# zhenpeiyang/RelativePose

Hardware: AMD Instinct MI355X
Metric: scan-pairs/sec end-to-end (completion+feat+spectral-match), 160x640 RGB-D (higher is better)
Workload: dtype f32 (fp32 products emulated on the bf16 matrix pipe: every operand cut into 3 bf16 pieces = its full 24 significand bits, the 6 partial products >= 2^-16 |ab| issued as v_mfma_f32_32x32x16_bf16, the 3 smallest dropped: a product error <= 2^-23 |ab| worst case, rms 2^-27.4 -- an fp32 multiply's own r

## Files before the change

include/relpose.h:

```cpp
#ifndef RELPOSE_H
#define RELPOSE_H

#include <stddef.h>
#include <stdint.h>

#ifdef __cplusplus
extern "C" {
#endif

#define RELPOSE_EINVAL (-1)
#define RELPOSE_ENOMEM (-2)
#define RELPOSE_EROUNDS (-3)

enum {
    RELPOSE_OK = 0,
    RELPOSE_FEW_KEYPOINTS = 1,
    RELPOSE_DIST_FILTER = 2,
    RELPOSE_ANGLE_FILTER = 3,
    RELPOSE_ZERO_WEIGHT = 4,
    RELPOSE_EDGE_OVERFLOW = 5,
    RELPOSE_NOT_CONVERGED = 6
};

enum { RELPOSE_SUNCG = 0, RELPOSE_MATTERPORT = 1, RELPOSE_SCANNET = 2 };
// ... 3 lines not shown

typedef struct RelposeParams {
    double distThre;
    double distSepThre;
    double angleThre;
    double sigmaAngle1, sigmaAngle2, sigmaDist, sigmaFeat;
    double mu;
    int32_t topK;
    int32_t method;
} RelposeParams;

void relpose_default_params(RelposeParams* p_host);

enum { RELPOSE_TUNE_AFFINITY_KERNEL = 0, RELPOSE_TUNE_FIT_MAX_PRODUCTS = 1, RELPOSE_TUNE_FIT_CLUSTER = 2,
       RELPOSE_TUNE_FIT_GLOBAL_VECTORS = 3, RELPOSE_TUNE_FIT_FIXED_CHECKS = 4, RELPOSE_TUNE_HEADS_KERNEL = 5, RELPOSE_TUNE_DECONV_STRIP = 6,
       RELPOSE_TUNE_ZERO_TILES = 7, RELPOSE_TUNE_CONV1_ZERO = 8, RELPOSE_TUNE_CONV4_ROWS = 9, RELPOSE_TUNE_COUNT = 10 };
int relpose_set_tuning(int32_t key, int32_t value);
const char* relpose_version(void);
typedef struct RelposeKeypoints {
    int32_t B, ns_max, nt_max;
    const int32_t* ns;
    const int32_t* nt;
    const double* pc_s;
    const double* normal_s;
    const float* feat_s;
    const double* weight_s;
    const double* pc_t;
    const double* normal_t;
    const float* feat_t;
    const double* weight_t;
} RelposeKeypoints;
// ... 716 lines not shown
} RelposeForwardArgs;
int relpose_scnet_forward_ex(RelposeSCNet* net, const RelposeForwardArgs* args);

int relpose_scnet_last_tail(RelposeSCNet* net);

int relpose_scnet_plan_macs(RelposeSCNet* net, int32_t n_images, int32_t flags, int32_t self_cached, double* macs_host);

int relpose_scnet_layer_kernel(RelposeSCNet* net, const char* layer, int32_t n_images);

int relpose_scnet_zero_tiles(RelposeSCNet* net, void* workspace, void* stream, int64_t* counts_host);

int relpose_scnet_conv1_zero(RelposeSCNet* net, void* workspace, void* stream, int64_t* counts_host, uint32_t* occ_host);

int relpose_scnet_conv4_rows(RelposeSCNet* net, void* workspace, void* stream, int64_t* counts_host);

int64_t relpose_scnet_read_tap(RelposeSCNet* net, const char* layer, float* out, void* workspace, void* stream);

int relpose_scnet_profile(RelposeSCNet* net, const float* x, float* out, int32_t n_images, int32_t H, int32_t W,
                          void* workspace, size_t workspace_bytes, int32_t iters,
                          double* ms_gemm_host, double* ms_other_host, int64_t* n_gemm_launches_host, void* stream);

#ifdef __cplusplus
}
#endif
#endif
```

relativepose_amd/_lib.py:

```python
import ctypes as C
import os

HERE = os.path.dirname(os.path.abspath(__file__))
LIB_PATH = os.environ.get("RELPOSE_LIB_PATH") or os.path.join(HERE, "librelpose_hip.so")

c_void_p, c_int, c_int64, c_size_t, c_double, c_char_p = C.c_void_p, C.c_int32, C.c_int64, C.c_size_t, C.c_double, C.c_char_p


class Params(C.Structure):
    _fields_ = [("distThre", c_double), ("distSepThre", c_double), ("angleThre", c_double),
                ("sigmaAngle1", c_double), ("sigmaAngle2", c_double), ("sigmaDist", c_double),
                ("sigmaFeat", c_double), ("mu", c_double), ("topK", c_int), ("method", c_int)]


class Keypoints(C.Structure):
    _fields_ = [("B", c_int), ("ns_max", c_int), ("nt_max", c_int),
                ("ns", c_void_p), ("nt", c_void_p),
                ("pc_s", c_void_p), ("normal_s", c_void_p), ("feat_s", c_void_p), ("weight_s", c_void_p),
                ("pc_t", c_void_p), ("normal_t", c_void_p), ("feat_t", c_void_p), ("weight_t", c_void_p)]


class MatchDebug(C.Structure):
    _fields_ = [("wij", c_void_p), ("corres_j", c_void_p), ("corres_w", c_void_p),
                ("counts", c_void_p), ("trace", c_void_p), ("eig_iters", c_void_p)]
# ... 301 lines not shown
    "relpose_scnet_create_ex": (c_void_p, [C.POINTER(SCNetConfig)]),
    "relpose_scnet_destroy": (None, [c_void_p]),
    "relpose_scnet_set_param": (c_int, [c_void_p, c_char_p, c_void_p, c_size_t]),
    "relpose_scnet_finalize": (c_int, [c_void_p]),
    "relpose_scnet_set_precision": (c_int, [c_void_p, c_int]),
    "relpose_scnet_num_params": (c_int64, [c_void_p]),
    "relpose_scnet_workspace_bytes": (c_size_t, [c_void_p, c_int, c_int, c_int]),
    "relpose_scnet_forward": (c_int, [c_void_p, c_void_p, c_void_p, c_int, c_int, c_int, c_void_p, c_size_t, c_void_p]),
    "relpose_scnet_forward_ex": (c_int, [c_void_p, C.POINTER(ForwardArgs)]),
    "relpose_scnet_plan_macs": (c_int, [c_void_p, c_int, c_int, c_int, C.POINTER(c_double)]),
    "relpose_scnet_layer_kernel": (c_int, [c_void_p, c_char_p, c_int]),
    "relpose_scnet_zero_tiles": (c_int, [c_void_p, c_void_p, c_void_p, C.POINTER(c_int64)]),
    "relpose_scnet_last_tail": (c_int, [c_void_p]),
    "relpose_scnet_conv1_zero": (c_int, [c_void_p, c_void_p, c_void_p, C.POINTER(c_int64), c_void_p]),
    "relpose_scnet_conv4_rows": (c_int, [c_void_p, c_void_p, c_void_p, C.POINTER(c_int64)]),
    "relpose_scnet_read_tap": (c_int64, [c_void_p, c_char_p, c_void_p, c_void_p, c_void_p]),
    "relpose_scnet_profile": (c_int, [c_void_p, c_void_p, c_void_p, c_int, c_int, c_int, c_void_p, c_size_t, c_int,
                                      C.POINTER(c_double), C.POINTER(c_double), C.POINTER(c_int64), c_void_p]),
}

_lib = None


def lib():
    global _lib
    if _lib is None:
        if not os.path.exists(LIB_PATH):
            _build_locked()
        if not os.path.exists(LIB_PATH):
            raise RuntimeError(f"{LIB_PATH} not built: run `python -m relativepose_amd.build` "
# ... 13 lines not shown
def _build_locked():
    import fcntl
    from . import build as _b
    if not os.path.exists(os.environ.get("HIPCC", "/opt/rocm/bin/hipcc")):
        return
    with open(LIB_PATH + ".lock", "w") as lk:
        fcntl.flock(lk, fcntl.LOCK_EX)
        try:
            if not os.path.exists(LIB_PATH):
                _b.build(verbose=False)
        finally:
            fcntl.flock(lk, fcntl.LOCK_UN)


TUNE_KEYS = {"affinity_kernel": 0, "fit_max_products": 1, "fit_cluster": 2, "fit_global_vectors": 3, "fit_fixed_checks": 4,
             "heads_kernel": 5, "deconv_strip": 6, "zero_tiles": 7, "conv1_zero": 8, "conv4_rows": 9}
AFFINITY_KERNELS = {"auto": 0, "rows": 1, "tile": 2, "lds": 3, "pool": 4}


class tuning:

    def __init__(self, **kw):
        self.kw = {k: (AFFINITY_KERNELS[v] if k == "affinity_kernel" and isinstance(v, str) else int(v)) for k, v in kw.items()}
        self.old = {}

    def __enter__(self):
        for k, v in self.kw.items():
            self.old[k] = lib().relpose_set_tuning(TUNE_KEYS[k], v)
        return self

    def __exit__(self, *exc):
# ... 25 lines not shown
```

relativepose_amd/csrc/scnet.hip:

```cpp
#include "common.h"
#include "matcher_internal.h"
#include "conv1_zero_geom.h"
#include "sample_pixels.h"
#include <map>
#include <string>
#include <vector>
#include <algorithm>
#include <math.h>
#include <stdio.h>
#include <string.h>
#include <type_traits>
#include <stdlib.h>
#include <stddef.h>

namespace {

typedef float floatx16 __attribute__((ext_vector_type(16)));
typedef __bf16 bf16x8 __attribute__((ext_vector_type(8)));
typedef __bf16 bf16x4 __attribute__((ext_vector_type(4)));
typedef _Float16 f16x8 __attribute__((ext_vector_type(8)));
typedef _Float16 f16x4 __attribute__((ext_vector_type(4)));
template <int SPLIT> struct SplitT { typedef bf16x8 v8; typedef bf16x4 v4; };
template <> struct SplitT<2> { typedef f16x8 v8; typedef f16x4 v4; };
template <> struct SplitT<3> { typedef f16x8 v8; typedef f16x4 v4; };
// ... 501 lines not shown
#pragma unroll
            for (int i = 0; i < MI; ++i)
#pragma unroll
                for (int j = 0; j < NI; ++j) {
                    acc[i][j] = __builtin_amdgcn_mfma_f32_32x32x2f32(a[i].x, b[j].x, acc[i][j], 0, 0, 0);
                    acc[i][j] = __builtin_amdgcn_mfma_f32_32x32x2f32(a[i].y, b[j].y, acc[i][j], 0, 0, 0);
                    acc[i][j] = __builtin_amdgcn_mfma_f32_32x32x2f32(a[i].z, b[j].z, acc[i][j], 0, 0, 0);
                    acc[i][j] = __builtin_amdgcn_mfma_f32_32x32x2f32(a[i].w, b[j].w, acc[i][j], 0, 0, 0);
                }
        }
    } else rp_split_mma<SPLIT, MI, NI>(acc, At, a_rows, Bt, b_rows);
}

#define RP_DT_SPLIT_OCC 2
#define RP_DT_OCC(MI_, NI_, NW_, SP_, PAIR_) ((SP_) >= 4 ? 2 : ((MI_) * (NI_) == 1 ? ((NW_) == 4 ? (((SP_) && (PAIR_)) ? RP_DT_SPLIT_OCC : 3) : 2) : 2))
template <int MI, int NI, int NW, int TC, bool PAIR = false, int SPLIT = 0>
__global__ __launch_bounds__(NW * 64, RP_DT_OCC(MI, NI, NW, SPLIT, PAIR)) void deconv_tile_kernel(const ConvDesc* __restrict__ descs) {
    constexpr int NT = NW * 64, TR = 32 / TC;
    constexpr int LD = RowLd<SPLIT>::v;
    constexpr bool S3 = SPLIT >= 4;
    constexpr int WB = S3 ? 6 : 4;
    constexpr int PR = PAIR ? 8 : (TC == 16 ? TR * MI * NW : TR), PW = PAIR ? 8 : (TC == 16 ? 16 : TC * NW), HW2 = PW + 2;
    constexpr int SUBPIX = (PR + 2) * HW2, NPIX = (PAIR ? 2 : 1) * SUBPIX;
    static_assert(TC == 16 || MI == 1, "strip layout: one tile per wave");
    static_assert(!PAIR || (TC == 8 && NW == 4 && MI == 1), "paired 8 x 8 patches: 4 waves of one 4 x 8 tile");
    constexpr int PSTEP = NT / KQ;
    constexpr int A_SLOTS = (NPIX + PSTEP - 1) / PSTEP;
    constexpr int B_ROWS = 4 * NI * 32;
    constexpr int B_SLOTS = (B_ROWS + PSTEP - 1) / PSTEP;
    static_assert(BK == 32, "one 128-byte line per pixel and chunk");
    __shared__ __attribute__((aligned(16))) float At[NPIX * LD];
    __shared__ __attribute__((aligned(16))) float Bt[4 * NI * 32 * LD];
// ... 222 lines not shown
                if (p == 3 && !last) RP_DT_STORE_A(c0n)
                __syncthreads();
            }
            if (snap_mode == 1 && ch + 1 == nch1) snap_store();
        }
    }
#undef RP_DT_LOAD_B2
#undef RP_DT_STORE_B2
#undef RP_DT_LOAD_A
#undef RP_DT_STORE_A
#undef RP_DT_LOAD_B
#undef RP_DT_STORE_B

    double* red = reinterpret_cast<double*>(&At[0]);
    const int patch = blockIdx.x;
#pragma unroll
    for (int p = 0; p < 4; ++p) {
        if constexpr (SPLIT == 2 || SPLIT == 3) {
            const float wsc = dh[p].wscale;
#pragma unroll
            for (int i = 0; i < MI; ++i)
#pragma unroll
                for (int j = 0; j < NI; ++j)
#pragma unroll
                    for (int r = 0; r < 16; ++r) acc[p][i][j][r] *= wsc;
        }
        if (dh[p].stat_part) {
#pragma unroll
            for (int j = 0; j < NI; ++j) {
                double sm = 0.0, sq = 0.0;
// ... 3 lines not shown
                    for (int r = 0; r < 16; ++r) { const double v = (double)acc[p][i][j][r]; sm += v; sq += v * v; }
                sm += rp_shfl_xor_d(sm, 32); sq += rp_shfl_xor_d(sq, 32);
                if (h == 0) { red[((wave * NI + j) * 32 + l31) * 2] = sm; red[((wave * NI + j) * 32 + l31) * 2 + 1] = sq; }
            }
            __syncthreads();
            if (tid < NI * 32) {
                double a = 0, b = 0;
#pragma unroll
                for (int w = 0; w < NW; ++w) { a += red[((w * NI) * 32 + tid) * 2]; b += red[((w * NI) * 32 + tid) * 2 + 1]; }
                double* o = dh[p].stat_part + (((size_t)patch * 2) * d.cout_pad + n0 + tid) * 2;
                rp_stg(o, a); rp_stg(o + 1, b);
            }
            __syncthreads();
        }
        const int opy = dh[p].py, opx = dh[p].px;
#pragma unroll
        for (int i = 0; i < MI; ++i)
#pragma unroll
            for (int r = 0; r < 16; ++r) {
                const int rl = (r & 3) + 8 * (r >> 2) + 4 * h;
                const int ry = try0 + TR * i + rl / TC, cx = tcx0 + rl % TC;
                const size_t pix = ((size_t)(wsp ? imgs[1] : imgs[0]) * d.Hout + 2 * ((wsp ? y0s[1] : y0s[0]) + ry) + opy) * d.Wout + 2 * ((wsp ? x0s[1] : x0s[0]) + cx) + opx;
                float* yo = d.y + pix * d.ycstride + d.ychoff + n0 + l31;
#pragma unroll
                for (int j = 0; j < NI; ++j)
                    if (n0 + j * 32 + l31 < d.Cout) rp_stg(yo + j * 32, acc[p][i][j][r]);
            }
    }
}

template <int MI, int NI, int TC, bool PAIR, int SPLIT = 0>
__global__ __launch_bounds__(256, SPLIT >= 4 ? 2 : (MI * NI <= 2 ? 4 : 3)) void conv_s2_tile_kernel(const ConvDesc* __restrict__ descs) {
    constexpr int NW = 4, NT = 256, TR = 32 / TC;
    constexpr int LD = RowLd<SPLIT>::v;
    constexpr bool S3 = SPLIT >= 4;
    constexpr int WB = S3 ? 6 : 4;
// ... 1396 lines not shown
        const int qp = PER * unit + sp, img = qp / ppi, prem = qp - img * ppi;
        const size_t pix = ((size_t)img * d.Hout + (prem / ppx) * PR + r) * d.Wout + (prem % ppx) * PW + c;
        return d.y + pix * d.ycstride + d.ychoff;
    };
    for (int i = tid; i < PER * PR * PW * c4n; i += 256) {
        const int c4 = i % c4n, pp = i / c4n, sp = pp / (PR * PW), lp = pp - sp * (PR * PW), r = lp / PW, c = lp - r * PW;
        const float4 v = *reinterpret_cast<const float4*>(at(f.y, sp, r, c) + 4 * c4);
        *reinterpret_cast<float4*>(at(f.x, sp, r, c) + 4 * c4) = v;
    }
    if (d.stat_part && tid < d.cout_pad) {
        const double2 v = *reinterpret_cast<const double2*>(d.stat_part + (((size_t)f.y * 2) * d.cout_pad + tid) * 2);
        *reinterpret_cast<double2*>(d.stat_part + (((size_t)f.x * 2) * d.cout_pad + tid) * 2) = v;
    }
}

__device__ __forceinline__ void lin_coef(int dst, float scale, int in, int& i0, int& i1, float& l0, float& l1) {
    float src = scale * (dst + 0.5f) - 0.5f;
    if (src < 0.f) src = 0.f;
    i0 = (int)src;
    if (i0 > in - 1) i0 = in - 1;
    i1 = i0 + ((i0 < in - 1) ? 1 : 0);
    l1 = src - i0;
    l0 = 1.f - l1;
}

__device__ __forceinline__ void resize_in_pixel(const float* __restrict__ x, float* __restrict__ y, size_t idx, int img, int oy, int ox, int H, int W,
                                                float shh, float sww, int c_begin, float (&out)[16]) {
    int y0, y1, x0, x1; float ly0, ly1, lx0, lx1;
    lin_coef(oy, shh, H, y0, y1, ly0, ly1);
    lin_coef(ox, sww, W, x0, x1, lx0, lx1);
#pragma unroll
    for (int c = 0; c < 16; ++c) {
        if (c < c_begin) continue;
        const float* p = x + ((size_t)img * 16 + c) * H * W;
        out[c] = ly0 * (lx0 * p[(size_t)y0 * W + x0] + lx1 * p[(size_t)y0 * W + x1]) +
                 ly1 * (lx0 * p[(size_t)y1 * W + x0] + lx1 * p[(size_t)y1 * W + x1]);
    }
    float4* o = reinterpret_cast<float4*>(y + idx * 16);
#pragma unroll
// ... 136 lines not shown

__global__ __launch_bounds__(256) void heads_sampled_kernel(const SampledDesc sd) {
    __shared__ float ndl[4][16][4];
    __shared__ float fl[4][16][32];
    const int lane = threadIdx.x & 63, wave = threadIdx.x >> 6;
    const int img = blockIdx.y, k = blockIdx.x * 4 + wave;
    if (k >= sd.npts_max || k >= sd.npts[img]) return;
    const int H = sd.H, W = sd.W, cf = sd.cf, feat_off = cf - 32;
    const double px = sd.pts[((size_t)img * sd.npts_max + k) * 2 + 0], py = sd.pts[((size_t)img * sd.npts_max + k) * 2 + 1];
    const RpSamplePix sp = rp_sample_pixels(px, py, H);
    const float shh = (float)RS / H, sww = (float)RS / W;
    const int g = img >> 1;
    const float2* ssd = sd.ss_d2 + (size_t)g * 224;
    const float2* ssa = sd.ss_a1 + (size_t)g * 192;
    auto item_src = [&](int item, int by, int bx, int& oy, int& ox, size_t& spix) {
        oy = by + (item >> 3); ox = bx + ((item >> 2) & 1);
        if (oy < 0 || oy >= H || ox < 0 || ox >= W) return false;
        int y0, y1, x0, x1; float ly0, ly1, lx0, lx1;
        lin_coef(oy, shh, RS, y0, y1, ly0, ly1);
        lin_coef(ox, sww, RS, x0, x1, lx0, lx1);
        spix = ((size_t)img * RS + ((item & 2) ? y1 : y0)) * RS + ((item & 1) ? x1 : x0);
        return true;
    };
    if (lane < 16) {
        int oy, ox; size_t spix;
        if (item_src(lane, sp.ty, sp.tx, oy, ox, spix)) {
            const float* pa = sd.a1 + spix * 192;
            const float* pd = sd.d2 + spix * 224;
            float an[3] = {0.f, 0.f, 0.f}, ad = 0.f;
            for (int c = 0; c < 32; ++c) {
                const float2 sc = ssa[64 + c];
                const float v = lrelu(pa[64 + c] * sc.x + sc.y, LRELU);
                for (int j = 0; j < 3; ++j) an[j] = __builtin_fmaf(v, sd.w[(128 + c) * 4 + j], an[j]);
            }
            for (int c = 0; c < 32; ++c) {
                const float2 sc = ssa[128 + c];
// ... 39 lines not shown
    const size_t hw = (size_t)H * W;
    float* const oi = sd.out + (size_t)img * cf * hw;
    for (int e = lane; e < 16 + 128; e += 64) {
        const bool nd = e < 16;
        const int p = nd ? (e >> 2) : ((e - 16) >> 5), c = nd ? (e & 3) : ((e - 16) & 31);
        const int oy = (nd ? sp.ty : sp.yi) + (p >> 1), ox = (nd ? sp.tx : sp.xi) + (p & 1);
        if (oy < 0 || oy >= H || ox < 0 || ox >= W) continue;
        int y0, y1, x0, x1; float ly0, ly1, lx0, lx1;
        lin_coef(oy, shh, RS, y0, y1, ly0, ly1);
        lin_coef(ox, sww, RS, x0, x1, lx0, lx1);
        const float a = nd ? ndl[wave][p * 4 + 0][c] : fl[wave][p * 4 + 0][c], b = nd ? ndl[wave][p * 4 + 1][c] : fl[wave][p * 4 + 1][c];
        const float cc = nd ? ndl[wave][p * 4 + 2][c] : fl[wave][p * 4 + 2][c], dd = nd ? ndl[wave][p * 4 + 3][c] : fl[wave][p * 4 + 3][c];
        const float r = __fmaf_rn(ly0, __fmaf_rn(lx0, a, __fmul_rn(lx1, b)), __fmul_rn(ly1, __fmaf_rn(lx0, cc, __fmul_rn(lx1, dd))));
        oi[(size_t)(nd ? 3 + c : feat_off + c) * hw + (size_t)oy * W + ox] = r;
    }
}

struct Phase {
    int ntaps; signed char offy[16], offx[16];
    int py, px, Hp, Wp;
    size_t w_off;
    size_t ws_off = 0;
    size_t wh_off = 0;
    float wh_scale = 1.f;
    size_t w3_off = 0;
    int K;
};

struct Layer {
    std::string name;
// ... 19 lines not shown
    int64_t nparams = 0;
    float* d_w = nullptr;
    float* d_gb = nullptr;
    float2* d_ident = nullptr;
    size_t w1_off = 0;
    size_t wh_off = 0, bh_off = 0;
    std::map<std::pair<void*, int64_t>, void*> plans;
    struct SelfState { uint64_t tag = 0, gen = 0; int n = 0, H = 0, W = 0; int snap_heads = 0; int heads_snap = 0; bool c4_rows = false; };
    std::map<void*, SelfState> self_state;
    std::map<std::string, Layer> layers;
    std::map<std::string, Buf> bufs;
    size_t per_image_floats = 0, ss_float2_per_group = 0;
    size_t gb_floats = 0;
    int last_n = 0;
    int last_tail = -1;
    const int* last_zt_counts = nullptr;
    const int* last_c4_hdr = nullptr;
    int last_c4_nimg[6] = {0, 0, 0, 0, 0, 0};
    int64_t last_zt_units[2] = {0, 0};
    bool w1_finite = false;
    struct A1zState { uint64_t gen = 0; int n = 0, H = 0, W = 0; };
    std::map<void*, A1zState> a1z_state;
    int64_t last_c1_units = 0;
    bool last_c1_codes = false, last_occ = false;
    bool profiling = false;
    std::vector<hipEvent_t> ev;
    std::vector<int> ev_kind;
};

namespace {
// ... 214 lines not shown
    if (b == "A8") return {P("conv8", 512)};
    if (b == "A9") return {P("conv9", 1024)};
    if (b == "D9") return {P("deconv9", 512)};
    if (b == "D8") return {P("deconv8", 512)};
    if (b == "D7") return {P("deconv7", 512)};
    if (b == "D6") return {P("deconv6", 512)};
    if (b == "D5") return {P("deconv5", 256)};
    if (b == "D4") return {P("deconv4", 128)};
    if (b == "D3") return {P("deconv3rgb", 64), P("deconv3n", 64), P("deconv3d", 64), P("deconv3s", 64), P("deconv3f", 64)};
    if (b == "D2") return {P("deconv2rgb", 32), P("deconv2n", 32), P("deconv2d", 32), P("deconv2s", 64), P("deconv2f", 64)};
    return {};
}

enum { OP_CONV = 0, OP_REDUCE = 1, OP_STATS = 2, OP_CONV1 = 3, OP_STATS_FUSED = 4, OP_HEADS = 5, OP_DECONV_TILE = 6, OP_CONV_S2 = 7, OP_CONV_STRIP = 8, OP_BCAST = 9, OP_NOP = 10, OP_SS_FILL = 11, OP_ZT_FILL = 12 };
struct Op { int type; int first, count, cfg; dim3 grid; std::string buf; int sslds = 0, uni = 0, split = 0; int ninner = 1, mt_max = 1; int skip_blk = 0; };

struct Plan {
    int n = 0; void* ws = nullptr;
    bool zero_warp = false;
    bool pose_only = false;
    bool self_cached = false;
    size_t persist_floats = 0;
    size_t snap_floats = 0;
    size_t heads_snap_off = 0;
    int snap_mode = 0;
    int snap_heads = 7;
    std::vector<ConvDesc> descs;
    std::vector<Op> ops;
    size_t splitk_floats = 0;
    size_t stat_doubles = 0;
    ConvDesc* d_descs = nullptr;
    int tail_first = -1;
    int head_count = 0;
    hipEvent_t tail_ev = nullptr, head_ev = nullptr;
    bool zt = false;
    int zt_nimg[6] = {0, 0, 0, 0, 0, 0};
    int64_t zt_units[2] = {0, 0};
    bool c4_rows = false;
    int c4_desc = -1, c4_skip = 0;
    int c4_nimg[6] = {0, 0, 0, 0, 0, 0};
};

struct Builder {
    RelposeSCNet* net; int n, G;
    float* act; float2* ss; float* splitk; double* statp;
    int pend_first = -1, pend_count = 0, pend_bm = 0; bool pend_ok = true;
    int pend_reduce = -1, pend_groups = 0;
    Plan* plan;
    int rc = 0;
    int group_first = -1;
    bool zero_warp = false;
    bool pose_only = false;
    bool self_cached = false;
    float* persist = nullptr;
    float* snapbuf = nullptr;
// ... 383 lines not shown
    one("deconv9", R.src("A9", 0, 1024), nullptr, 1, "D9", 0); R.stats("D9");
    sk = R.src("A8", 0, 512); one("deconv8", R.src("D9", 0, 512), skp, 3, "D8", 0); R.stats("D8");
    sk = R.src("A7", 0, 512); one("deconv7", R.src("D8", 0, 512), skp, 3, "D7", 0); R.stats("D7");
    sk = R.src("A6", 0, 512); one("deconv6", R.src("D7", 0, 512), skp, 7, "D6", 0); R.stats("D6");
    sk = R.src("A5", 0, 512); one("deconv5", R.src("D6", 0, 512), skp, 14, "D5", 0); R.stats("D5");
    sk = R.src("A4", 0, 256); one("deconv4", R.src("D5", 0, 256), skp, 28, "D4", 0); R.stats("D4");
    auto wanted = [&](int m) { return ((net->omask >> m) & 1) && (!R.pose_only || (m != 0 && m != 3)); };
    R.begin_group();
    for (int m = 0; m < 5; ++m) {
        if (!wanted(m)) continue;
        if (m < 3) { sk = R.src("A3", 2 * m * 128, 128); R.head_of[(int)R.plan->descs.size()] = m; R.conv(std::string("deconv3") + heads[m], R.src("D4", 0, 128), &sk, 56, "D3", m * 64); }
        else R.conv(std::string("deconv3") + heads[m], R.src("D4", 0, 128), nullptr, 56, "D3", m * 64);
    }
    R.end_group(); R.stats("D3");
    const int d2off[5] = {0, 32, 64, 96, 160};
    R.begin_group();
    for (int m = 0; m < 3; ++m) if (wanted(m)) { sk = R.src("A2", 2 * m * 64, 64); R.head_of[(int)R.plan->descs.size()] = m; R.conv(std::string("deconv2") + heads[m], R.src("D3", m * 64, 64), &sk, 112, "D2", d2off[m]); }
    R.end_group();
    R.begin_group();
    for (int m = 3; m < 5; ++m) if (wanted(m)) R.conv(std::string("deconv2") + heads[m], R.src("D3", m * 64, 64), nullptr, 112, "D2", d2off[m]);
    R.end_group(); R.stats("D2");
    R.plan->tail_first = (int)R.plan->ops.size();
    if (net->S != 15 && net->S != 21) {
        if (R.pose_only) R.rc = RELPOSE_EINVAL;
        const int ooff[5] = {0, 3, 6, 7, 7 + net->S};
        for (int cp = 32; cp <= 64; cp *= 2) {
            R.begin_group();
            for (int m = 0; m < 5; ++m) {
                const auto L = net->layers.find(std::string("deconv1") + heads[m]);
                if (!wanted(m) || L == net->layers.end() || L->second.cout_pad != cp) continue;
                if (m < 3) { sk = R.src("A1", 2 * m * 32, 32); R.conv(std::string("deconv1") + heads[m], R.src("D2", d2off[m], 32), &sk, 224, "OUT", ooff[m]); }
                else R.conv(std::string("deconv1") + heads[m], R.src("D2", d2off[m], 64), nullptr, 224, "OUT", ooff[m]);
            }
            R.end_group();
        }
    } else {
// ... 11 lines not shown
}

void free_plan(RelposeSCNet* net) {
    for (auto& kv : net->plans) {
        Plan* p = (Plan*)kv.second;
        if (p->d_descs) (void)hipFree(p->d_descs);
        if (p->tail_ev) (void)hipEventDestroy(p->tail_ev);
        if (p->head_ev) (void)hipEventDestroy(p->head_ev);
        delete p;
    }
    net->plans.clear();
    net->self_state.clear();
    net->a1z_state.clear();
}

struct WsOffsets { size_t act, ss, partial, splitk, statp, persist, snap, zt, c4r, total; };

WsOffsets ws_offsets(RelposeSCNet* net, int n) {
    Plan dry;
    Builder B; B.net = net; B.n = n; B.G = n / 2; B.act = nullptr; B.ss = nullptr; B.splitk = nullptr; B.statp = nullptr; B.plan = &dry;
    build_plan(net, n, B);
    WsOffsets o;
    size_t off = 0;
    o.act = off; off += rp_align(net->per_image_floats * n * sizeof(float));
    o.ss = off; off += rp_align(net->ss_float2_per_group * (n / 2) * sizeof(float2));
    o.partial = off; off += rp_align(partial_doubles(n / 2) * sizeof(double));
    o.splitk = off; off += rp_align(dry.splitk_floats * sizeof(float));
    o.statp = off; off += rp_align(dry.stat_doubles * sizeof(double));
    o.persist = off; off += rp_align(dry.persist_floats * sizeof(float));
    o.snap = off; off += rp_align(dry.snap_floats * sizeof(float));
    o.zt = off; off += rp_align(zt_ints(n) * sizeof(int));
    o.c4r = off; off += rp_align(c4r_ints(n) * sizeof(int));
    o.total = off;
    return o;
}

}

extern "C" {

RelposeSCNet* relpose_scnet_create(int32_t snumclass, int32_t use_tanh) {
    if (snumclass < 1 || snumclass > 64) return nullptr;
    RelposeSCNet* net = new RelposeSCNet();
    net->S = snumclass; net->use_tanh = use_tanh; net->cf = 7 + snumclass + 32;
    return net;
}

// ... 281 lines not shown
        mark(2);
        if (!occ_fused)
            hipLaunchKernelGGL(x0_occupancy_kernel, dim3(n * ZT_NB), dim3(256), 0, s, act + net->bufs["X0"].off * n, occ, ztp, plan->self_cached ? 8 : 0);
        hipLaunchKernelGGL(zero_tile_list_kernel, dim3(G, 6, 2), dim3(128), 0, s, occ, ztp, zm, n * ZT_PPI);
        if (plan->c4_rows) {
            const ConvDesc& d4 = plan->descs[plan->c4_desc];
            ZtMembers cm;
            for (int q = 0; q < 6; ++q) cm.nimg[q] = plan->c4_nimg[q];
            hipLaunchKernelGGL(conv4_row_list_kernel, dim3(G, 6), dim3(256), 0, s, occ, cm, G, const_cast<int*>(d4.c4_cnt), const_cast<int*>(d4.c4_list),
                               const_cast<int*>(d4.c4_map));
            net->last_c4_hdr = d4.c4_hdr;
            for (int q = 0; q < 6; ++q) net->last_c4_nimg[q] = plan->c4_nimg[q];
        }
        mark(-2);
        net->last_zt_counts = ztp;
    }
    int op_index = -1;
    for (const Op& op : plan->ops) {
        ++op_index;
        if (op.type == OP_NOP) continue;
        if (op_index == plan->head_count && s != (hipStream_t)stream) {
            if (!plan->head_ev) RP_HIP(hipEventCreateWithFlags(&plan->head_ev, hipEventDisableTiming));
            RP_HIP(hipEventRecord(plan->head_ev, s));
            s = (hipStream_t)stream;
            RP_HIP(hipStreamWaitEvent(s, plan->head_ev, 0));
        }
        if (op_index == plan->tail_first && two) {
            if (!plan->tail_ev) RP_HIP(hipEventCreateWithFlags(&plan->tail_ev, hipEventDisableTiming));
            RP_HIP(hipEventRecord(plan->tail_ev, s));
            s = (hipStream_t)tail_stream;
// ... 71 lines not shown
            mark(1);
#define RP_L_S2A(SP_) hipLaunchKernelGGL((conv_s2_tile_kernel<2, 2, 16, false, SP_>), op.grid, dim3(256), 0, s, plan->d_descs + op.first)
#define RP_L_S2C(SP_) hipLaunchKernelGGL((conv_s2_tile_kernel<1, 4, 8, true, SP_>), op.grid, dim3(256), 0, s, plan->d_descs + op.first)
            if (op.cfg == 0) RP_TILE_SPLIT(RP_L_S2A);
            else RP_TILE_SPLIT(RP_L_S2C);
#undef RP_L_S2A
#undef RP_L_S2C
            mark(-1);
        } else if (op.type == OP_ZT_FILL) {
            mark(2);
            if (op.cfg == 0) hipLaunchKernelGGL((zero_tile_fill_kernel<false>), op.grid, dim3(256), 0, s, plan->d_descs + op.first);
            else hipLaunchKernelGGL((zero_tile_fill_kernel<true>), op.grid, dim3(256), 0, s, plan->d_descs + op.first);
            mark(-2);
        } else if (op.type == OP_DECONV_TILE) {
            mark(1);
#define RP_L_DT1(SP_) hipLaunchKernelGGL((deconv_tile_kernel<1, 2, 4, 16, false, SP_>), op.grid, dim3(256), 0, s, plan->d_descs + op.first)
#define RP_L_DT2(SP_) hipLaunchKernelGGL((deconv_tile_kernel<1, 1, 4, 16, false, SP_>), op.grid, dim3(256), 0, s, plan->d_descs + op.first)
#define RP_L_DT4(SP_) hipLaunchKernelGGL((deconv_tile_kernel<1, 1, 4, 8, true, SP_>), op.grid, dim3(256), 0, s, plan->d_descs + op.first)
            if (op.cfg == 1) {
                if (op.split == 2) RP_L_DT1(2);
                else if (op.split == 3) RP_L_DT1(3);
                else if (op.split >= 4) return RELPOSE_EINVAL;
                else RP_L_DT1(0);
            }
            else if (op.cfg == 2) RP_TILE_SPLIT(RP_L_DT2);
            else RP_TILE_SPLIT(RP_L_DT4);
#undef RP_L_DT1
#undef RP_L_DT2
#undef RP_L_DT4
#undef RP_TILE_SPLIT
            mark(-1);
        } else if (op.type == OP_CONV1) {
            mark(1);
            hipLaunchKernelGGL(conv1_mfma_kernel, dim3(196 * n), dim3(256), 0, s, act + net->bufs["X0"].off * n, net->d_w + net->w1_off,
                               act + net->bufs["A1"].off * n, partial, n, (plan->zero_warp ? 1 : 0) | (plan->self_cached ? 2 : 0),
                               c1z ? (const unsigned*)occ : nullptr, a1z, zcode);
            net->last_c1_units = (int64_t)C1Z_TILES * (plan->self_cached ? 3 * n : (plan->zero_warp ? 3 * n + 3 * 2 : 6 * n));
            net->last_c1_codes = c1z;
            mark(-1);
        } else if (op.type == OP_STATS_FUSED) {
            const Buf& B = net->bufs[op.buf];
            mark(2);
            hipLaunchKernelGGL(bn_finalize_fused_kernel, dim3((B.C + 31) / 32, G), dim3(1024), 0, s, plan->d_descs + op.first, op.count, op.skip_blk,
                               B.C, 2 * B.H * B.H, net->d_gb + B.gb_off, net->d_gb + B.gb_off + B.C, ssp + B.ss_off * G);
// ... 194 lines not shown
    }
    const char* lo = (const char*)workspace + ws_offsets(net, net->last_n).c4r;
    if ((const char*)net->last_c4_hdr != lo) return RELPOSE_EINVAL;
    int h[12];
    RP_HIP(hipMemcpyAsync(h, net->last_c4_hdr, sizeof(h), hipMemcpyDeviceToHost, (hipStream_t)stream));
    RP_HIP(hipStreamSynchronize((hipStream_t)stream));
    for (int q = 0; q < 6; ++q) {
        const int64_t rows = (int64_t)net->last_c4_nimg[q] * C4R_HW;
        if (rows == 0) continue;
        const bool lp = h[2 * q + 1] != 0;
        counts_host[3 * q] = lp ? h[2 * q] : rows; counts_host[3 * q + 1] = lp ? rows - h[2 * q] : 0; counts_host[3 * q + 2] = lp ? 1 : 0;
    }
    return 0;
}

int relpose_scnet_conv1_zero(RelposeSCNet* net, void* workspace, void* stream, int64_t* counts_host, uint32_t* occ_host) {
    if (!net || !net->finalized || !workspace || !counts_host || net->last_n <= 0) return RELPOSE_EINVAL;
    const int n = net->last_n;
    counts_host[0] = net->last_c1_units; counts_host[1] = 0; counts_host[2] = 0;
    if (occ_host && !net->last_occ) return RELPOSE_EINVAL;
    const int* base = (const int*)((const char*)workspace + ws_offsets(net, n).zt);
    std::vector<unsigned short> codes;
    if (net->last_c1_codes) {
        codes.resize((size_t)n * C1Z_TILES);
        const unsigned char* a1z = (const unsigned char*)(base + zt_list_ints(n));
        RP_HIP(hipMemcpyAsync(codes.data(), a1z + c1z_state_bytes(n), codes.size() * sizeof(unsigned short), hipMemcpyDeviceToHost, (hipStream_t)stream));
    }
    if (occ_host) RP_HIP(hipMemcpyAsync(occ_host, base, zt_occ_ints(n) * sizeof(uint32_t), hipMemcpyDeviceToHost, (hipStream_t)stream));
    RP_HIP(hipStreamSynchronize((hipStream_t)stream));
    int64_t launched = 0;
// ... 49 lines not shown
```

relativepose_amd/model.py:

```python
import ctypes as C

import numpy as np
import torch

from . import _lib
from .weights import HEADS, head_channels, parse_output_type, state_dict_spec

PRECISION_CODES = {"f32": 0, "bf16x3": 1, "f16x3": 2, "f16": 3, "bf16x9": 4, "bf16x6": 5}

BUFFER_SHAPES = {"X0": (224, 16), "A1": (224, 192), "A2": (112, 384), "A3": (56, 768), "A4": (28, 256), "A5": (14, 512),
                 "A6": (7, 512), "A7": (3, 512), "A8": (3, 512), "A9": (1, 1024), "D9": (3, 512), "D8": (3, 512),
                 "D7": (7, 512), "D6": (14, 512), "D5": (28, 256), "D4": (56, 128), "D3": (112, 320), "D2": (224, 224)}


_REGISTRY = {}


class SCNet(torch.nn.Module):

    def __init__(self, args):
        super().__init__()
        self.snumclass = int(args.snumclass)
        self.useTanh = int(getattr(args, "useTanh", 1))
        self.batchnorm = int(bool(getattr(args, "batchnorm", 1)))
# ... 147 lines not shown
            out = torch.empty(n, self.out_channels, H, W, dtype=torch.float32, device=x.device)
            if tail_stream is not None:
                out.record_stream(tail_stream)
        else:
            assert out.is_cuda and out.dtype == torch.float32 and out.is_contiguous() and tuple(out.shape) == (n, self.out_channels, H, W)
        a = _lib.ForwardArgs()
        a.struct_size = C.sizeof(_lib.ForwardArgs)
        a.flags = int(flags) & (7 | self.FLAG_SAMPLED_OUTPUTS)
        if a.flags & self.FLAG_SAMPLED_OUTPUTS:
            if sample_pts is None or sample_npts is None:
                raise ValueError("RELPOSE_FWD_SAMPLED_OUTPUTS needs sample_pts and sample_npts")
            assert sample_pts.is_cuda and sample_pts.dtype == torch.float64 and sample_pts.is_contiguous() and sample_pts.dim() == 3
            assert tuple(sample_pts.shape) == (n, sample_pts.shape[1], 2) and sample_pts.shape[1] > 0
            assert sample_npts.is_cuda and sample_npts.dtype == torch.int32 and sample_npts.is_contiguous() and tuple(sample_npts.shape) == (n,)
            a.sample_pts, a.sample_npts, a.sample_npts_max = sample_pts.data_ptr(), sample_npts.data_ptr(), int(sample_pts.shape[1])
            if tail_stream is not None:
                sample_pts.record_stream(tail_stream)
                sample_npts.record_stream(tail_stream)
        a.x, a.out = x.data_ptr(), out.data_ptr()
        a.n_images, a.H, a.W = n, H, W
        a.workspace, a.workspace_bytes = ws.data_ptr(), ws.numel()
        a.stream = torch.cuda.current_stream().cuda_stream
        a.tail_stream = a.stream if tail_stream is None else tail_stream.cuda_stream
        a.self_tag = int(self_tag)
        a.workspace_generation = self._ws_gen
        _lib.check(_lib.lib().relpose_scnet_forward_ex(self._h, C.byref(a)), "relpose_scnet_forward_ex")
        if self.is_variant:
            sel = out if self.out_channels == self.full_channels else out[:, self._sel]
            if user_out is None:
                return sel.contiguous()
            user_out.copy_(sel)
            return user_out
        return out
# ... 19 lines not shown
        import numpy as np
        v = (C.c_int64 * 3)()
        occ = np.zeros((self._ws_n, 6, 28), np.uint32) if occupancy else None
        _lib.check(_lib.lib().relpose_scnet_conv1_zero(self._h, _lib.ptr(self._ws), _lib.stream_ptr(), v,
                                                       occ.ctypes.data_as(C.c_void_p) if occupancy else None), "relpose_scnet_conv1_zero")
        counts = (int(v[0]), int(v[1]), int(v[2]))
        return (counts, occ.astype(np.int64)) if occupancy else counts

    def conv4_rows(self):
        v = (C.c_int64 * 18)()
        _lib.check(_lib.lib().relpose_scnet_conv4_rows(self._h, _lib.ptr(self._ws), _lib.stream_ptr(), v), "relpose_scnet_conv4_rows")
        if v[0] < 0:
            return None
        return [(int(v[3 * q]), int(v[3 * q + 1]), bool(v[3 * q + 2])) for q in range(6)]

    def layer_on_strip_kernel(self, layer, n):
        return self.layer_kernel(layer, n) in (1, 2)

    def read_tap(self, name):
        import torch
        L = _lib.lib()
        cnt = L.relpose_scnet_read_tap(self._h, name.encode(), None, None, None)
        if cnt < 0:
            raise KeyError(name)
        H, Cc = BUFFER_SHAPES[name] if name != "OUT" else (224, self.full_channels)
        out = torch.empty(cnt, dtype=torch.float32, device=self._ws.device)
        L.relpose_scnet_read_tap(self._h, name.encode(), _lib.ptr(out), _lib.ptr(self._ws), _lib.stream_ptr())
        return out.view(-1, H, H, Cc)

    def profile(self, x, iters=3):
# ... 10 lines not shown
```

Before: 1114.

## Mask deconv2 output stores to pixels read by sampled-output bilinear taps

Adds a per-image bitmask kernel that marks which 224x224 D2 pixels the sampled-output bilinear resampling will read, then launches masked variants of the deconv2 tile kernel that skip stores (and whole sub-pixel phases) for unmarked pixels. The aim is to cut the D2 write traffic when only sparse keypoint outputs are needed. It adds one small kernel launch and workspace, relies on the plan check that downstream consumers only read the sampled pixels, and leaves unwritten D2 values stale, which could matter if anything else (such as the D2 stats) reads the full buffer.

```diff
diff --git a/include/relpose.h b/include/relpose.h
--- a/include/relpose.h
+++ b/include/relpose.h
@@ -41,7 +41,7 @@
 
 enum { RELPOSE_TUNE_AFFINITY_KERNEL = 0, RELPOSE_TUNE_FIT_MAX_PRODUCTS = 1, RELPOSE_TUNE_FIT_CLUSTER = 2,
        RELPOSE_TUNE_FIT_GLOBAL_VECTORS = 3, RELPOSE_TUNE_FIT_FIXED_CHECKS = 4, RELPOSE_TUNE_HEADS_KERNEL = 5, RELPOSE_TUNE_DECONV_STRIP = 6,
-       RELPOSE_TUNE_ZERO_TILES = 7, RELPOSE_TUNE_CONV1_ZERO = 8, RELPOSE_TUNE_CONV4_ROWS = 9, RELPOSE_TUNE_COUNT = 10 };
+       RELPOSE_TUNE_ZERO_TILES = 7, RELPOSE_TUNE_CONV1_ZERO = 8, RELPOSE_TUNE_CONV4_ROWS = 9, RELPOSE_TUNE_D2_MASK = 10, RELPOSE_TUNE_COUNT = 11 };
 int relpose_set_tuning(int32_t key, int32_t value);
 const char* relpose_version(void);
 typedef struct RelposeKeypoints {
@@ -788,6 +788,8 @@
 
 int relpose_scnet_conv4_rows(RelposeSCNet* net, void* workspace, void* stream, int64_t* counts_host);
 
+int relpose_scnet_d2_mask(RelposeSCNet* net, void* workspace, void* stream, int64_t* counts_host, uint32_t* mask_host);
+
 int64_t relpose_scnet_read_tap(RelposeSCNet* net, const char* layer, float* out, void* workspace, void* stream);
 
 int relpose_scnet_profile(RelposeSCNet* net, const float* x, float* out, int32_t n_images, int32_t H, int32_t W,
diff --git a/relativepose_amd/_lib.py b/relativepose_amd/_lib.py
--- a/relativepose_amd/_lib.py
+++ b/relativepose_amd/_lib.py
@@ -339,6 +339,7 @@
     "relpose_scnet_last_tail": (c_int, [c_void_p]),
     "relpose_scnet_conv1_zero": (c_int, [c_void_p, c_void_p, c_void_p, C.POINTER(c_int64), c_void_p]),
     "relpose_scnet_conv4_rows": (c_int, [c_void_p, c_void_p, c_void_p, C.POINTER(c_int64)]),
+    "relpose_scnet_d2_mask": (c_int, [c_void_p, c_void_p, c_void_p, C.POINTER(c_int64), c_void_p]),
     "relpose_scnet_read_tap": (c_int64, [c_void_p, c_char_p, c_void_p, c_void_p, c_void_p]),
     "relpose_scnet_profile": (c_int, [c_void_p, c_void_p, c_void_p, c_int, c_int, c_int, c_void_p, c_size_t, c_int,
                                       C.POINTER(c_double), C.POINTER(c_double), C.POINTER(c_int64), c_void_p]),
@@ -382,7 +383,8 @@
 
 
 TUNE_KEYS = {"affinity_kernel": 0, "fit_max_products": 1, "fit_cluster": 2, "fit_global_vectors": 3, "fit_fixed_checks": 4,
-             "heads_kernel": 5, "deconv_strip": 6, "zero_tiles": 7, "conv1_zero": 8, "conv4_rows": 9}
+             "heads_kernel": 5, "deconv_strip": 6, "zero_tiles": 7, "conv1_zero": 8, "conv4_rows": 9,
+             "d2_mask": 10}
 AFFINITY_KERNELS = {"auto": 0, "rows": 1, "tile": 2, "lds": 3, "pool": 4}
 
 
diff --git a/relativepose_amd/csrc/sample_src_pixels.h b/relativepose_amd/csrc/sample_src_pixels.h
--- /dev/null
+++ b/relativepose_amd/csrc/sample_src_pixels.h
@@ -0,0 +1,24 @@
+#pragma once
+#include "sample_pixels.h"
+
+__device__ __forceinline__ void lin_coef(int dst, float scale, int in, int& i0, int& i1, float& l0, float& l1) {
+    float src = scale * (dst + 0.5f) - 0.5f;
+    if (src < 0.f) src = 0.f;
+    i0 = (int)src;
+    if (i0 > in - 1) i0 = in - 1;
+    i1 = i0 + ((i0 < in - 1) ? 1 : 0);
+    l1 = src - i0;
+    l0 = 1.f - l1;
+}
+
+constexpr int RP_SRC_ITEMS = 16;
+
+__device__ __forceinline__ bool rp_sample_src_pixel(int item, int by, int bx, int H, int W, int rs, float shh, float sww, int& oy, int& ox, int& sy, int& sx) {
+    oy = by + (item >> 3); ox = bx + ((item >> 2) & 1);
+    if (oy < 0 || oy >= H || ox < 0 || ox >= W) return false;
+    int y0, y1, x0, x1; float ly0, ly1, lx0, lx1;
+    lin_coef(oy, shh, rs, y0, y1, ly0, ly1);
+    lin_coef(ox, sww, rs, x0, x1, lx0, lx1);
+    sy = (item & 2) ? y1 : y0; sx = (item & 1) ? x1 : x0;
+    return true;
+}
diff --git a/relativepose_amd/csrc/scnet.hip b/relativepose_amd/csrc/scnet.hip
--- a/relativepose_amd/csrc/scnet.hip
+++ b/relativepose_amd/csrc/scnet.hip
@@ -2,6 +2,7 @@
 #include "matcher_internal.h"
 #include "conv1_zero_geom.h"
 #include "sample_pixels.h"
+#include "sample_src_pixels.h"
 #include <map>
 #include <string>
 #include <vector>
@@ -539,8 +540,9 @@
 
 #define RP_DT_SPLIT_OCC 2
 #define RP_DT_OCC(MI_, NI_, NW_, SP_, PAIR_) ((SP_) >= 4 ? 2 : ((MI_) * (NI_) == 1 ? ((NW_) == 4 ? (((SP_) && (PAIR_)) ? RP_DT_SPLIT_OCC : 3) : 2) : 2))
-template <int MI, int NI, int NW, int TC, bool PAIR = false, int SPLIT = 0>
-__global__ __launch_bounds__(NW * 64, RP_DT_OCC(MI, NI, NW, SPLIT, PAIR)) void deconv_tile_kernel(const ConvDesc* __restrict__ descs) {
+template <int MI, int NI, int NW, int TC, bool PAIR = false, int SPLIT = 0, bool MASKED = false>
+__global__ __launch_bounds__(NW * 64, RP_DT_OCC(MI, NI, NW, SPLIT, PAIR)) void deconv_tile_kernel(const ConvDesc* __restrict__ descs, const unsigned* __restrict__ d2m) {
+    static_assert(!MASKED || (TC == 16 && !PAIR && MI == 1), "masked stores: the 8 x 16 patch, whose output rows are whole mask words");
     constexpr int NT = NW * 64, TR = 32 / TC;
     constexpr int LD = RowLd<SPLIT>::v;
     constexpr bool S3 = SPLIT >= 4;
@@ -793,6 +795,13 @@
 
     double* red = reinterpret_cast<double*>(&At[0]);
     const int patch = blockIdx.x;
+    unsigned mrow[MASKED ? TR : 1][2];
+    if constexpr (MASKED) {
+        const int wpr = d.Wout >> 5;
+        const unsigned* mp = d2m + ((size_t)imgs[0] * d.Hout + 2 * (y0s[0] + TR * __builtin_amdgcn_readfirstlane(wave))) * wpr + (x0s[0] >> 4);
+#pragma unroll
+        for (int a = 0; a < TR; ++a) { mrow[a][0] = mp[(2 * a) * wpr]; mrow[a][1] = mp[(2 * a + 1) * wpr]; }
+    }
 #pragma unroll
     for (int p = 0; p < 4; ++p) {
         if constexpr (SPLIT == 2 || SPLIT == 3) {
@@ -826,12 +835,22 @@
             __syncthreads();
         }
         const int opy = dh[p].py, opx = dh[p].px;
+        unsigned mph[MASKED ? TR : 1];
+        if constexpr (MASKED) {
+            unsigned any = 0u;
+#pragma unroll
+            for (int a = 0; a < TR; ++a) { const unsigned w = opy ? mrow[a][1] : mrow[a][0]; any |= w; mph[a] = w >> (8 * h + opx); }
+            if (!any) continue;
+        }
 #pragma unroll
         for (int i = 0; i < MI; ++i)
 #pragma unroll
             for (int r = 0; r < 16; ++r) {
                 const int rl = (r & 3) + 8 * (r >> 2) + 4 * h;
                 const int ry = try0 + TR * i + rl / TC, cx = tcx0 + rl % TC;
+                if constexpr (MASKED) {
+                    if (!((mph[r >> 3] >> (2 * (((r & 3) + 8 * (r >> 2)) % TC))) & 1u)) continue;
+                }
                 const size_t pix = ((size_t)(wsp ? imgs[1] : imgs[0]) * d.Hout + 2 * ((wsp ? y0s[1] : y0s[0]) + ry) + opy) * d.Wout + 2 * ((wsp ? x0s[1] : x0s[0]) + cx) + opx;
                 float* yo = d.y + pix * d.ycstride + d.ychoff + n0 + l31;
 #pragma unroll
@@ -2258,15 +2277,6 @@
     }
 }
 
-__device__ __forceinline__ void lin_coef(int dst, float scale, int in, int& i0, int& i1, float& l0, float& l1) {
-    float src = scale * (dst + 0.5f) - 0.5f;
-    if (src < 0.f) src = 0.f;
-    i0 = (int)src;
-    if (i0 > in - 1) i0 = in - 1;
-    i1 = i0 + ((i0 < in - 1) ? 1 : 0);
-    l1 = src - i0;
-    l0 = 1.f - l1;
-}
 
 __device__ __forceinline__ void resize_in_pixel(const float* __restrict__ x, float* __restrict__ y, size_t idx, int img, int oy, int ox, int H, int W,
                                                 float shh, float sww, int c_begin, float (&out)[16]) {
@@ -2433,12 +2443,9 @@
     const float2* ssd = sd.ss_d2 + (size_t)g * 224;
     const float2* ssa = sd.ss_a1 + (size_t)g * 192;
     auto item_src = [&](int item, int by, int bx, int& oy, int& ox, size_t& spix) {
-        oy = by + (item >> 3); ox = bx + ((item >> 2) & 1);
-        if (oy < 0 || oy >= H || ox < 0 || ox >= W) return false;
-        int y0, y1, x0, x1; float ly0, ly1, lx0, lx1;
-        lin_coef(oy, shh, RS, y0, y1, ly0, ly1);
-        lin_coef(ox, sww, RS, x0, x1, lx0, lx1);
-        spix = ((size_t)img * RS + ((item & 2) ? y1 : y0)) * RS + ((item & 1) ? x1 : x0);
+        int sy, sx;
+        if (!rp_sample_src_pixel(item, by, bx, H, W, RS, shh, sww, oy, ox, sy, sx)) return false;
+        spix = ((size_t)img * RS + sy) * RS + sx;
         return true;
     };
     if (lane < 16) {
@@ -2508,6 +2515,30 @@
         const float r = __fmaf_rn(ly0, __fmaf_rn(lx0, a, __fmul_rn(lx1, b)), __fmul_rn(ly1, __fmaf_rn(lx0, cc, __fmul_rn(lx1, dd))));
         oi[(size_t)(nd ? 3 + c : feat_off + c) * hw + (size_t)oy * W + ox] = r;
     }
+}
+
+constexpr int D2M_WPR = RS / 32, D2M_WORDS = RS * D2M_WPR;
+static_assert(RS % 32 == 0, "a mask row is whole words");
+inline size_t d2m_ints(int n) { return (size_t)n * D2M_WORDS; }
+
+__global__ __launch_bounds__(256) void d2_mask_kernel(const double* __restrict__ pts, const int* __restrict__ npts, int npts_max, int H, int W,
+                                                      unsigned* __restrict__ mask) {
+    __shared__ unsigned m[D2M_WORDS];
+    const int img = blockIdx.x, tid = threadIdx.x;
+    for (int i = tid; i < D2M_WORDS; i += 256) m[i] = 0u;
+    __syncthreads();
+    const int np = min(npts[img], npts_max);
+    const float shh = (float)RS / H, sww = (float)RS / W;
+    for (long long e = tid; e < (long long)np * 2 * RP_SRC_ITEMS; e += 256) {
+        const int k = (int)(e / (2 * RP_SRC_ITEMS)), blk = (int)(e / RP_SRC_ITEMS) & 1, item = (int)(e % RP_SRC_ITEMS);
+        const double px = pts[((size_t)img * npts_max + k) * 2 + 0], py = pts[((size_t)img * npts_max + k) * 2 + 1];
+        const RpSamplePix sp = rp_sample_pixels(px, py, H);
+        int oy, ox, sy, sx;
+        if (rp_sample_src_pixel(item, blk ? sp.yi : sp.ty, blk ? sp.xi : sp.tx, H, W, RS, shh, sww, oy, ox, sy, sx))
+            atomicOr(&m[sy * D2M_WPR + (sx >> 5)], 1u << (sx & 31));
+    }
+    __syncthreads();
+    for (int i = tid; i < D2M_WORDS; i += 256) mask[(size_t)img * D2M_WORDS + i] = m[i];
 }
 
 struct Phase {
@@ -2557,6 +2588,7 @@
     size_t gb_floats = 0;
     int last_n = 0;
     int last_tail = -1;
+    bool last_d2_masked = false;
     const int* last_zt_counts = nullptr;
     const int* last_c4_hdr = nullptr;
     int last_c4_nimg[6] = {0, 0, 0, 0, 0, 0};
@@ -2801,6 +2833,7 @@
 
 enum { OP_CONV = 0, OP_REDUCE = 1, OP_STATS = 2, OP_CONV1 = 3, OP_STATS_FUSED = 4, OP_HEADS = 5, OP_DECONV_TILE = 6, OP_CONV_S2 = 7, OP_CONV_STRIP = 8, OP_BCAST = 9, OP_NOP = 10, OP_SS_FILL = 11, OP_ZT_FILL = 12 };
 struct Op { int type; int first, count, cfg; dim3 grid; std::string buf; int sslds = 0, uni = 0, split = 0; int ninner = 1, mt_max = 1; int skip_blk = 0; };
+constexpr bool rp_d2_mask_split(int split) { return split == 0 || (split >= 2 && split <= 5); }
 
 struct Plan {
     int n = 0; void* ws = nullptr;
@@ -2826,6 +2859,8 @@
     bool c4_rows = false;
     int c4_desc = -1, c4_skip = 0;
     int c4_nimg[6] = {0, 0, 0, 0, 0, 0};
+    int d2_first = 0, d2_end = 0;
+    bool d2_maskable = false;
 };
 
 struct Builder {
@@ -3239,12 +3274,22 @@
     }
     R.end_group(); R.stats("D3");
     const int d2off[5] = {0, 32, 64, 96, 160};
+    R.plan->d2_first = (int)R.plan->ops.size();
     R.begin_group();
     for (int m = 0; m < 3; ++m) if (wanted(m)) { sk = R.src("A2", 2 * m * 64, 64); R.head_of[(int)R.plan->descs.size()] = m; R.conv(std::string("deconv2") + heads[m], R.src("D3", m * 64, 64), &sk, 112, "D2", d2off[m]); }
     R.end_group();
     R.begin_group();
     for (int m = 3; m < 5; ++m) if (wanted(m)) R.conv(std::string("deconv2") + heads[m], R.src("D3", m * 64, 64), nullptr, 112, "D2", d2off[m]);
-    R.end_group(); R.stats("D2");
+    R.end_group();
+    R.plan->d2_end = (int)R.plan->ops.size();
+    R.stats("D2");
+    R.plan->d2_maskable = !R.rc && !net->variant() && R.plan->ops.back().type == OP_STATS_FUSED && R.plan->d2_end > R.plan->d2_first;
+    for (int i = R.plan->d2_first; i < R.plan->d2_end && R.plan->d2_maskable; ++i) {
+        const Op& o = R.plan->ops[i];
+        R.plan->d2_maskable = o.type == OP_DECONV_TILE && (o.cfg == 1 || o.cfg == 2) && rp_d2_mask_split(o.split) && !(o.cfg == 1 && o.split >= 4);
+        for (int k = o.first; k < o.first + o.count && R.plan->d2_maskable; ++k)
+            R.plan->d2_maskable = R.plan->descs[k].Hout == RS && R.plan->descs[k].Wout == RS;
+    }
     R.plan->tail_first = (int)R.plan->ops.size();
     if (net->S != 15 && net->S != 21) {
         if (R.pose_only) R.rc = RELPOSE_EINVAL;
@@ -3286,7 +3331,7 @@
     net->a1z_state.clear();
 }
 
-struct WsOffsets { size_t act, ss, partial, splitk, statp, persist, snap, zt, c4r, total; };
+struct WsOffsets { size_t act, ss, partial, splitk, statp, persist, snap, zt, c4r, d2m, total; };
 
 WsOffsets ws_offsets(RelposeSCNet* net, int n) {
     Plan dry;
@@ -3303,6 +3348,7 @@
     o.snap = off; off += rp_align(dry.snap_floats * sizeof(float));
     o.zt = off; off += rp_align(zt_ints(n) * sizeof(int));
     o.c4r = off; off += rp_align(c4r_ints(n) * sizeof(int));
+    o.d2m = off; off += rp_align(d2m_ints(n) * sizeof(unsigned));
     o.total = off;
     return o;
 }
@@ -3614,6 +3660,14 @@
         }
         mark(-2);
         net->last_zt_counts = ztp;
+    }
+    unsigned* const d2m = (unsigned*)(ws + o.d2m);
+    const bool d2_masked = sampled && plan->d2_maskable && g_rp_tune[RELPOSE_TUNE_D2_MASK] != 1;
+    net->last_d2_masked = d2_masked;
+    if (d2_masked) {
+        mark(2);
+        hipLaunchKernelGGL(d2_mask_kernel, dim3((unsigned)n), dim3(256), 0, s, args->sample_pts, args->sample_npts, args->sample_npts_max, H, W, d2m);
+        mark(-2);
     }
     int op_index = -1;
     for (const Op& op : plan->ops) {
@@ -3715,20 +3769,26 @@
             mark(-2);
         } else if (op.type == OP_DECONV_TILE) {
             mark(1);
-#define RP_L_DT1(SP_) hipLaunchKernelGGL((deconv_tile_kernel<1, 2, 4, 16, false, SP_>), op.grid, dim3(256), 0, s, plan->d_descs + op.first)
-#define RP_L_DT2(SP_) hipLaunchKernelGGL((deconv_tile_kernel<1, 1, 4, 16, false, SP_>), op.grid, dim3(256), 0, s, plan->d_descs + op.first)
-#define RP_L_DT4(SP_) hipLaunchKernelGGL((deconv_tile_kernel<1, 1, 4, 8, true, SP_>), op.grid, dim3(256), 0, s, plan->d_descs + op.first)
+#define RP_L_DT1(SP_) hipLaunchKernelGGL((deconv_tile_kernel<1, 2, 4, 16, false, SP_>), op.grid, dim3(256), 0, s, plan->d_descs + op.first, nullptr)
+#define RP_L_DT2(SP_) hipLaunchKernelGGL((deconv_tile_kernel<1, 1, 4, 16, false, SP_>), op.grid, dim3(256), 0, s, plan->d_descs + op.first, nullptr)
+#define RP_L_DT4(SP_) hipLaunchKernelGGL((deconv_tile_kernel<1, 1, 4, 8, true, SP_>), op.grid, dim3(256), 0, s, plan->d_descs + op.first, nullptr)
+#define RP_L_DT1M(SP_) hipLaunchKernelGGL((deconv_tile_kernel<1, 2, 4, 16, false, SP_, true>), op.grid, dim3(256), 0, s, plan->d_descs + op.first, d2m)
+#define RP_L_DT2M(SP_) hipLaunchKernelGGL((deconv_tile_kernel<1, 1, 4, 16, false, SP_, true>), op.grid, dim3(256), 0, s, plan->d_descs + op.first, d2m)
+            const bool msk = d2_masked && op_index >= plan->d2_first && op_index < plan->d2_end;
             if (op.cfg == 1) {
-                if (op.split == 2) RP_L_DT1(2);
+                if (op.split >= 4) return RELPOSE_EINVAL;
+                if (msk) { if (op.split == 2) RP_L_DT1M(2); else if (op.split == 3) RP_L_DT1M(3); else RP_L_DT1M(0); }
+                else if (op.split == 2) RP_L_DT1(2);
                 else if (op.split == 3) RP_L_DT1(3);
-                else if (op.split >= 4) return RELPOSE_EINVAL;
                 else RP_L_DT1(0);
             }
-            else if (op.cfg == 2) RP_TILE_SPLIT(RP_L_DT2);
+            else if (op.cfg == 2) { if (msk) RP_TILE_SPLIT(RP_L_DT2M); else RP_TILE_SPLIT(RP_L_DT2); }
             else RP_TILE_SPLIT(RP_L_DT4);
 #undef RP_L_DT1
 #undef RP_L_DT2
 #undef RP_L_DT4
+#undef RP_L_DT1M
+#undef RP_L_DT2M
 #undef RP_TILE_SPLIT
             mark(-1);
         } else if (op.type == OP_CONV1) {
@@ -3953,6 +4013,21 @@
     return 0;
 }
 
+int relpose_scnet_d2_mask(RelposeSCNet* net, void* workspace, void* stream, int64_t* counts_host, uint32_t* mask_host) {
+    if (!net || !net->finalized || !workspace || !counts_host || net->last_n <= 0) return RELPOSE_EINVAL;
+    const int n = net->last_n;
+    counts_host[0] = -1; counts_host[1] = (int64_t)n * RS * RS;
+    if (!net->last_d2_masked) return mask_host ? RELPOSE_EINVAL : 0;
+    std::vector<uint32_t> m(d2m_ints(n));
+    RP_HIP(hipMemcpyAsync(m.data(), (const char*)workspace + ws_offsets(net, n).d2m, m.size() * sizeof(uint32_t), hipMemcpyDeviceToHost, (hipStream_t)stream));
+    RP_HIP(hipStreamSynchronize((hipStream_t)stream));
+    int64_t bits = 0;
+    for (uint32_t w : m) bits += __builtin_popcount(w);
+    counts_host[0] = bits;
+    if (mask_host) memcpy(mask_host, m.data(), m.size() * sizeof(uint32_t));
+    return 0;
+}
+
 int relpose_scnet_conv1_zero(RelposeSCNet* net, void* workspace, void* stream, int64_t* counts_host, uint32_t* occ_host) {
     if (!net || !net->finalized || !workspace || !counts_host || net->last_n <= 0) return RELPOSE_EINVAL;
     const int n = net->last_n;
diff --git a/relativepose_amd/model.py b/relativepose_amd/model.py
--- a/relativepose_amd/model.py
+++ b/relativepose_amd/model.py
@@ -185,9 +185,10 @@
             assert tuple(sample_pts.shape) == (n, sample_pts.shape[1], 2) and sample_pts.shape[1] > 0
             assert sample_npts.is_cuda and sample_npts.dtype == torch.int32 and sample_npts.is_contiguous() and tuple(sample_npts.shape) == (n,)
             a.sample_pts, a.sample_npts, a.sample_npts_max = sample_pts.data_ptr(), sample_npts.data_ptr(), int(sample_pts.shape[1])
-            if tail_stream is not None:
-                sample_pts.record_stream(tail_stream)
-                sample_npts.record_stream(tail_stream)
+            for s_ in (torch.cuda.current_stream(), tail_stream):
+                if s_ is not None:
+                    sample_pts.record_stream(s_)
+                    sample_npts.record_stream(s_)
         a.x, a.out = x.data_ptr(), out.data_ptr()
         a.n_images, a.H, a.W = n, H, W
         a.workspace, a.workspace_bytes = ws.data_ptr(), ws.numel()
@@ -237,6 +238,20 @@
             return None
         return [(int(v[3 * q]), int(v[3 * q + 1]), bool(v[3 * q + 2])) for q in range(6)]
 
+    def d2_mask(self, mask=False):
+        import numpy as np
+        v = (C.c_int64 * 2)()
+        words = np.zeros((self._ws_n, 224, 7), np.uint32) if mask else None
+        L = _lib.lib()
+        _lib.check(L.relpose_scnet_d2_mask(self._h, _lib.ptr(self._ws), _lib.stream_ptr(), v, None), "relpose_scnet_d2_mask")
+        if v[0] < 0:
+            return None
+        if mask:
+            _lib.check(L.relpose_scnet_d2_mask(self._h, _lib.ptr(self._ws), _lib.stream_ptr(), v, words.ctypes.data_as(C.c_void_p)), "relpose_scnet_d2_mask")
+            bits = ((words[..., None] >> np.arange(32, dtype=np.uint32)) & 1).astype(bool).reshape(self._ws_n, 224, 224)
+            return (int(v[0]), int(v[1])), bits
+        return int(v[0]), int(v[1])
+
     def layer_on_strip_kernel(self, layer, n):
         return self.layer_kernel(layer, n) in (1, 2)
 
```

Result: no change. 1124 (median of 6 runs) (+0.8%).
